# CHAINNEVERLIU/Pytorch-RL-EnhancedStableBaselines

Measured on AMD Instinct MI355X. Metric: env-steps/sec (SAC, two-series CSTR, 4096 vec-envs) at 1/2/4/8 GPUs, higher is better.
Workload: dtype f32; 1 GPU; SAC MlpPolicy class defaults on 4096 vectorised two-series CSTR envs per GPU (obs 4/act 2, euler, batch 256, ring 244x4096, 1 gradient step per vec-step; hipGraph replay, 8 iterations per graph); n_envs_per_gpu=4096, global_batch=256, parallelism=dp1, hip_graph=True, hip_graph_requested=True, graph_unroll=8, blas=rocblas, n_updates=2370

## Files before the change

### pytorch-rl-enhancedstablebaselines_amd/csrc/cstr_chain.hip

```cpp
#include <hip/hip_runtime.h>
#include <stdint.h>

#include "../../include/cstr_rl_hip.h"
#include "cstr_device.h"
#include "cstr_rng_device.h"

namespace {

using f32x4 = __attribute__((ext_vector_type(4))) float;
typedef unsigned int u32x4 __attribute__((ext_vector_type(4)));
constexpr int BUF_OOB = 0x40000000;
constexpr int CH_THREADS = 256, CH_WAVES = 4;
constexpr float LOG_STD_MIN = -20.0f, LOG_STD_MAX = 2.0f;
constexpr int MAX_A = CSTR_MAX_HEAD_ACT;

constexpr int SM_PART = 0;
constexpr int SM_RED = SM_PART + 3 * 64 * 4;
constexpr int SM_XS = SM_RED + 4 * 16 * 8;
constexpr int SM_GS = SM_XS + 16 * 16;
constexpr int SM_PANEL = SM_GS + 16 * 8;
static size_t chain_lds_bytes(int k, int w1_pad) { return (size_t)(SM_PANEL + 16 * (k + 4) + w1_pad * k) * sizeof(float); }

__device__ __forceinline__ __amdgpu_buffer_rsrc_t rsrc_of(const float *base, const int64_t floats)
{
// ... 60 lines not shown
    const bool col_ok = k0 + r < K;
#pragma unroll
    for (int u = 0; u < NQ; ++u) {
        const int n = 16 * (ks + S * u) + 4 * h;
        const int wo = 4 * (n * K + k0 + r);
        bq[u].x = ld32(rw, (col_ok && n < N) ? wo : BUF_OOB);
        bq[u].y = ld32(rw, (col_ok && n + 1 < N) ? wo + 4 * K : BUF_OOB);
        bq[u].z = ld32(rw, (col_ok && n + 2 < N) ? wo + 8 * K : BUF_OOB);
        bq[u].w = ld32(rw, (col_ok && n + 3 < N) ? wo + 12 * K : BUF_OOB);
    }
}

template <int NQ>
__device__ __forceinline__ f32x4 tile_mma(const float *panel, const int ld, const int kdim, const float4 (&bq)[NQ], const int ks, const int S)
{
    const int lane = threadIdx.x & 63, r = lane & 15, h = lane >> 4;
    f32x4 acc0 = {0.0f, 0.0f, 0.0f, 0.0f}, acc1 = acc0, acc2 = acc0, acc3 = acc0;
    float4 av[NQ];
#pragma unroll
    for (int u = 0; u < NQ; ++u) {
        const int k = 16 * (ks + S * u) + 4 * h;
        av[u] = make_float4(0.0f, 0.0f, 0.0f, 0.0f);
        if (k < kdim) av[u] = *reinterpret_cast<const float4 *>(panel + r * ld + k);
    }
#pragma unroll
    for (int u = 0; u < NQ; ++u) {
        if (16 * (ks + S * u) < kdim) {
            acc0 = __builtin_amdgcn_mfma_f32_16x16x4f32(av[u].x, bq[u].x, acc0, 0, 0, 0);
            acc1 = __builtin_amdgcn_mfma_f32_16x16x4f32(av[u].y, bq[u].y, acc1, 0, 0, 0);
            acc2 = __builtin_amdgcn_mfma_f32_16x16x4f32(av[u].z, bq[u].z, acc2, 0, 0, 0);
            acc3 = __builtin_amdgcn_mfma_f32_16x16x4f32(av[u].w, bq[u].w, acc3, 0, 0, 0);
        }
    }
    return (acc0 + acc1) + (acc2 + acc3);
}

__device__ __forceinline__ f32x4 combine_split_k(f32x4 acc, float *smem, const int T, const int S)
{
    const int lane = threadIdx.x & 63, wave = threadIdx.x >> 6;
    f32x4 *part = reinterpret_cast<f32x4 *>(smem + SM_PART);
    if (S > 1) {
        if (wave >= T) part[(wave - T) * 64 + lane] = acc;
        lds_barrier();
        if (wave < T) {
            for (int v = 1; v < S; ++v) acc += part[(wave + T * v - T) * 64 + lane];
        }
    }
    return acc;
}

constexpr int MAX_PARTS = 16;
template <int NP>
__device__ __forceinline__ float sum_parts_n(const __amdgpu_buffer_rsrc_t rs, const int n, const int64_t stride, const int64_t at)
{
    float v[NP];
#pragma unroll
    for (int p = 0; p < NP; ++p) v[p] = ld32(rs, p < n ? (int)(4 * (p * stride + at)) : BUF_OOB);
    float s = v[0];
#pragma unroll
    for (int p = 1; p < NP; ++p) s += v[p];
    return s;
}

struct PartBatch {
    float v[8];
    const float *part; int n; int64_t stride, at, total;
    __device__ __forceinline__ void request(const float *part_, const int n_, const int64_t stride_, const int64_t at_, const int64_t total_)
    {
        part = part_; n = n_; stride = stride_; at = at_; total = total_;
        const __amdgpu_buffer_rsrc_t rs = rsrc_of(part, total);
#pragma unroll
        for (int p = 0; p < 8; ++p) v[p] = ld32(rs, (p < n && n <= 8) ? (int)(4 * (p * stride + at)) : BUF_OOB);
    }
    __device__ __forceinline__ float sum() const;
};

__device__ __forceinline__ float sum_parts(const float *part, const int n, const int64_t stride, const int64_t at, const int64_t total_floats)
{
    const __amdgpu_buffer_rsrc_t rs = rsrc_of(part, total_floats);
    if (n <= 4) return sum_parts_n<4>(rs, n, stride, at);
    if (n <= 8) return sum_parts_n<8>(rs, n, stride, at);
    if (n <= MAX_PARTS) return sum_parts_n<MAX_PARTS>(rs, n, stride, at);
    float s = part[at];
    for (int p = 1; p < n; ++p) s += part[p * stride + at];
    return s;
}

__device__ __forceinline__ float PartBatch::sum() const
{
    if (n > 8) return sum_parts(part, n, stride, at, total);
    float s = v[0];
#pragma unroll
    for (int p = 1; p < 8; ++p) s += v[p];
    return s;
}

__device__ __forceinline__ void sample_action(const float mu, const float raw, const float e, float &a, float &lp_term)
{
    const float half_log_2pi = 0.91893853320467274178f;
    const float ls = fminf(fmaxf(raw, LOG_STD_MIN), LOG_STD_MAX);
    const float sd = expf(ls);
    const float u = mu + sd * e;
    a = tanhf(u);
    const float d = u - mu, var = sd * sd;
    lp_term = (-(d * d) / (2.0f * var) - logf(sd) - half_log_2pi) - logf(1.0f - a * a + 1e-6f);
}

template <int KIN>
constexpr int l1_pad() { return (KIN % 2 == 0 && KIN + 1 <= 16) ? 0 : (KIN + 1 <= 8 ? 8 : 16); }
template <int KIN>
constexpr bool l1_bias_in_k() { return KIN % 4 != 0; }

template <int KIN>
__device__ __forceinline__ float4 l1_direct_quad(const float *w1, const float *b1, const int n, const int h, float &bias)
{
    if (KIN % 4 == 0) {
        bias = b1[n];
        return 4 * h < KIN ? *reinterpret_cast<const float4 *>(w1 + (int64_t)n * KIN + 4 * h) : make_float4(0.0f, 0.0f, 0.0f, 0.0f);
    }
    bias = 0.0f;
    const int k0 = 4 * h;
    float2 lo = make_float2(0.0f, 0.0f), hi = lo;
    if (k0 + 1 < KIN) lo = *reinterpret_cast<const float2 *>(w1 + (int64_t)n * KIN + k0);
    else if (k0 == KIN) lo = make_float2(b1[n], 0.0f);
    if (k0 + 3 < KIN) hi = *reinterpret_cast<const float2 *>(w1 + (int64_t)n * KIN + k0 + 2);
    else if (k0 + 2 == KIN) hi = make_float2(b1[n], 0.0f);
    return make_float4(lo.x, lo.y, hi.x, hi.y);
}

template <int KIN>
__device__ __forceinline__ void stage_w1(float *w1s, const float *w1, const float *b1, const int h1)
{
    constexpr int KP = l1_pad<KIN>();
    if (KP == 0) return;
    for (int c = threadIdx.x; c < h1; c += CH_THREADS) {
        float w[KP > 0 ? KP : 4];
#pragma unroll
        for (int k = 0; k < KP; ++k) w[k] = k < KIN ? w1[(int64_t)c * KIN + k] : 0.0f;
        w[KP > 0 ? KIN : 0] = b1[c];
#pragma unroll
        for (int q = 0; q < KP / 4; ++q) *reinterpret_cast<float4 *>(w1s + c * KP + 4 * q) = make_float4(w[4 * q], w[4 * q + 1], w[4 * q + 2], w[4 * q + 3]);
    }
}

template <int KIN>
struct L1Direct {
    float4 wb[4];
    float bias[4];
    __device__ __forceinline__ void request(const float *w1, const float *b1, const int h1)
    {
        const int lane = threadIdx.x & 63, wave = threadIdx.x >> 6, r = lane & 15, h = lane >> 4;
#pragma unroll
        for (int i = 0; i < 4; ++i) wb[i] = l1_direct_quad<KIN>(w1, b1, min(16 * (wave + CH_WAVES * i) + r, h1 - 1), h, bias[i]);
    }
};

template <int KP, int KIN>
__device__ __forceinline__ void layer1_mfma(const float *xs, const float *w1s, float *panel, const int ld, const int h1,
                                            const L1Direct<KIN> *dir = nullptr, const float *w1 = nullptr, const float *b1 = nullptr)
{
    const int lane = threadIdx.x & 63, wave = threadIdx.x >> 6, r = lane & 15, h = lane >> 4;
    const bool hk = KP == 0 ? 4 * h < KIN + (l1_bias_in_k<KIN>() ? 1 : 0) : 4 * h < KP;
    const float4 zero4 = make_float4(0.0f, 0.0f, 0.0f, 0.0f);
    const float4 xa = hk ? *reinterpret_cast<const float4 *>(xs + r * 16 + 4 * h) : zero4;
    const int n_tiles = (h1 + 15) / 16;
    for (int t0 = wave; t0 < n_tiles; t0 += 4 * CH_WAVES) {
        float4 wb[4];
        float bb[4] = {0.0f, 0.0f, 0.0f, 0.0f};
#pragma unroll
        for (int i = 0; i < 4; ++i) {
            if (KP == 0) {
                if (t0 == wave) { wb[i] = dir->wb[i]; bb[i] = dir->bias[i]; }
                else wb[i] = l1_direct_quad<KIN>(w1, b1, min(16 * (t0 + CH_WAVES * i) + r, h1 - 1), h, bb[i]);
            } else {
                wb[i] = hk ? *reinterpret_cast<const float4 *>(w1s + min(16 * (t0 + CH_WAVES * i) + r, h1 - 1) * KP + 4 * h) : zero4;
            }
        }
        f32x4 acc0[4], acc1[4];
#pragma unroll
        for (int i = 0; i < 4; ++i) {
            acc0[i] = {0.0f, 0.0f, 0.0f, 0.0f};
            acc1[i] = acc0[i];
            acc0[i] = __builtin_amdgcn_mfma_f32_16x16x4f32(xa.x, wb[i].x, acc0[i], 0, 0, 0);
            acc1[i] = __builtin_amdgcn_mfma_f32_16x16x4f32(xa.y, wb[i].y, acc1[i], 0, 0, 0);
        }
#pragma unroll
        for (int i = 0; i < 4; ++i) {
            acc0[i] = __builtin_amdgcn_mfma_f32_16x16x4f32(xa.z, wb[i].z, acc0[i], 0, 0, 0);
            acc1[i] = __builtin_amdgcn_mfma_f32_16x16x4f32(xa.w, wb[i].w, acc1[i], 0, 0, 0);
        }
#pragma unroll
        for (int i = 0; i < 4; ++i) {
            const int tl = t0 + CH_WAVES * i;
            const f32x4 acc = acc0[i] + acc1[i];
            if (tl < n_tiles && 16 * tl + r < h1) {
#pragma unroll
                for (int e = 0; e < 4; ++e) panel[(4 * h + e) * ld + 16 * tl + r] = fmaxf(acc[e] + bb[i], 0.0f);
            }
        }
    }
}

__device__ __forceinline__ void store_panel(const float *panel, const int ld, float *out, const int width, const int m0)
{
    const int qpr = width / 4;
    for (int i = threadIdx.x; i < 16 * qpr; i += CH_THREADS) {
        const int row = i / qpr, q = i % qpr;
        *reinterpret_cast<float4 *>(out + (int64_t)(m0 + row) * width + 4 * q) = *reinterpret_cast<const float4 *>(panel + row * ld + 4 * q);
    }
}

struct ActorFwdArgs {
    cstr_sac_actor_t net;
    cstr_ring_t ring; int64_t *ring_ctl; int advance_ring;
    const int32_t *idx; int batch, tiles;
    float *x_data, *x_pi, *x_next, *out_done, *out_rew, *a_h1, *a_h2, *head_part;
    const uint64_t *head_rng_ctl; uint64_t head_rng_offset; float *eps_all;
    int rows_mode, head_n;
};

template <int D, int A, int NQ, int WX>
__global__ __launch_bounds__(CH_THREADS) void sac_actor_chain_fwd_kernel(const ActorFwdArgs a)
{
    extern __shared__ __align__(16) float smem[];
    constexpr int W = D + A, QPR = D / 4;
    const int t = threadIdx.x, lane = t & 63, wave = t >> 6, r = lane & 15, h = lane >> 4;
    const int T = WX ? exact_tiles<NQ, WX>() : a.tiles, S = CH_WAVES / T, tile = wave % T, ks = wave / T;
    const int H1 = WX ? exact_h1<WX>() : a.net.h1, H2 = WX ? exact_h2<WX>() : a.net.h2, B = a.batch, mode = a.rows_mode, HN = a.head_n;
    const int M = mode == CSTR_CHAIN_ROWS_PAIR ? 2 * B : B;
    const int n0 = (blockIdx.x * T + tile) * 16, m0 = blockIdx.y * 16;
    float *xs = smem + SM_XS, *red = smem + SM_RED, *panel = smem + SM_PANEL;
    const int ld = H1 + 4;
    float *w1s = panel + 16 * ld;
    const bool col_ok = n0 + r < H2;
    CH_STAMP(0, 0);
    float4 bq[NQ];
    load_b_fwd<NQ>(bq, a.net.w2, H2, H1, n0, ks, S);
    const int col = min(n0 + r, H2 - 1);
    const float bv = a.net.b2[col];
    float hwv[2 * A];
#pragma unroll
    for (int j = 0; j < 2 * A; ++j) hwv[j] = j < HN ? a.net.hw[(int64_t)j * H2 + col] : 0.0f;
    stage_w1<D>(w1s, a.net.w1, a.net.b1, H1);
    L1Direct<D> l1d;
    if (l1_pad<D>() == 0) l1d.request(a.net.w1, a.net.b1, H1);
    const bool mat = a.idx != nullptr && blockIdx.x == 0;
    float4 v = make_float4(0.0f, 0.0f, 0.0f, 0.0f), vo = v;
    float actv[A], dn = 0.0f, to = 0.0f, rw = 0.0f;
#pragma unroll
    for (int j = 0; j < A; ++j) actv[j] = 0.0f;
    int b = 0;
    bool next = false;
    const bool data_row = mode != CSTR_CHAIN_ROWS_PAIR;
    if (t < 16 * QPR) {
        const int row = t / QPR, qd = t % QPR, m = m0 + row;
        next = mode == CSTR_CHAIN_ROWS_PAIR ? m >= B : mode == CSTR_CHAIN_ROWS_NEXT;
        b = (mode == CSTR_CHAIN_ROWS_PAIR && next) ? m - B : m;
        if (a.idx) {
            const int64_t o = (int64_t)a.idx[b] * a.ring.n_envs + a.idx[B + b];
            v = *reinterpret_cast<const float4 *>((next ? a.ring.next_obs : a.ring.obs) + o * D + 4 * qd);
            if (mat && data_row && next) vo = *reinterpret_cast<const float4 *>(a.ring.obs + o * D + 4 * qd);
            if (mat && (!next || data_row) && qd == 0) {
#pragma unroll
                for (int j = 0; j < A; ++j) actv[j] = a.ring.act[o * A + j];
                dn = a.ring.done[o]; to = a.ring.timeout[o]; rw = a.ring.rew[o];
            }
        } else {
            const float2 *src = reinterpret_cast<const float2 *>((next ? a.x_next : a.x_pi) + (int64_t)b * W + 4 * qd);
            const float2 lo = src[0], hi = src[1];
            v = make_float4(lo.x, lo.y, hi.x, hi.y);
        }
        *reinterpret_cast<float4 *>(xs + row * 16 + 4 * qd) = v;
    } else if (t >= 64 && t < 64 + 16 * (4 - QPR)) {
        const int i = t - 64, row = i / (4 - QPR), qd = QPR + i % (4 - QPR);
        *reinterpret_cast<float4 *>(xs + row * 16 + 4 * qd) = make_float4(qd == QPR ? 1.0f : 0.0f, 0.0f, 0.0f, 0.0f);
    }
    constexpr int PAIRS = (A + 1) / 2;
    float e0 = 0.0f, e1 = 0.0f;
    const bool noise = a.eps_all != nullptr && blockIdx.x == 0 && wave == 3 && lane < 16 * PAIRS;
    if (noise) {
        const int row = lane / PAIRS, pr = lane % PAIRS;
        const uint64_t seed = a.head_rng_ctl[0], ctr = a.head_rng_ctl[1] + a.head_rng_offset + (uint64_t)(m0 + row);
        uint32_t rr[4];
        philox4x32_10((uint32_t)ctr, (uint32_t)(ctr >> 32), (uint32_t)pr, 0u, (uint32_t)seed, (uint32_t)(seed >> 32), rr);
        box_muller(rr[0], rr[1], e0, e1);
    }
    CH_STAMP(0, 1);
    lds_barrier();
    CH_STAMP(0, 2);
    layer1_mfma<l1_pad<D>(), D>(xs, w1s, panel, ld, H1, &l1d, a.net.w1, a.net.b1);
    lds_barrier();
    CH_STAMP(0, 3);
    f32x4 acc = tile_mma<NQ>(panel, ld, H1, bq, ks, S);
    CH_STAMP(0, 4);
    acc = combine_split_k(acc, smem, T, S);
    CH_STAMP(0, 5);
    float hv[4] = {0.0f, 0.0f, 0.0f, 0.0f};
    if (wave < T) {
#pragma unroll
        for (int e = 0; e < 4; ++e) hv[e] = col_ok ? fmaxf(acc[e] + bv, 0.0f) : 0.0f;
#pragma unroll
        for (int j = 0; j < 2 * A; ++j) {
            if (j < HN) {
#pragma unroll
                for (int e = 0; e < 4; ++e) {
                    const float s = rowsum16(hv[e] * hwv[j]);
// ... 786 lines not shown
#pragma unroll
        for (int e = 0; e < 4; ++e) d[e] = (col_ok && ty[e] > 0.0f) ? acc[e] : 0.0f;
        if (GACT) {
#pragma unroll
            for (int j = 0; j < A; ++j) {
#pragma unroll
                for (int e = 0; e < 4; ++e) {
                    const float s = rowsum16(d[e] * w1a[j]);
                    if (r == 0) red[(tile * 16 + 4 * h + e) * 8 + j] = s;
                }
            }
        }
    }
    if (GACT) {
        lds_barrier();
        if (t < 16 * A) {
            const int row = t / A, j = t % A;
            float s = red[row * 8 + j];
#pragma unroll
            for (int tl = 1; tl < T; ++tl) s += red[(tl * 16 + row) * 8 + j];
            o_gact[(((int64_t)g * gridDim.x + blockIdx.x) * B + m0 + row) * A + j] = s;
        }
    }
    CH_STAMP(2, 6);
    if (!GACT) {
        if (wave < T && col_ok) {
#pragma unroll
            for (int e = 0; e < 4; ++e) o_dz1[((int64_t)g * B + m0 + 4 * h + e) * H1 + k0 + r] = d[e];
        }
        const int cpg = (H2 + gridDim.x - 1) / gridDim.x;
        if (t / cpg == (int)blockIdx.x) {
#pragma unroll
            for (int row = 0; row < 16; ++row) o_dz2[((int64_t)g * B + m0 + row) * H2 + t] = y[row];
        }
    }
    if (t < 16 && blockIdx.x == 0) {
        const int row = m0 + t;
        if (o_q) o_q[(int64_t)g * B + row] = o_qv;
        if (o_gqp) o_gqp[(int64_t)g * B + row] = o_gq;
        if (MODE == 1 && g == 0 && o_tqp) o_tqp[row] = o_tq;
    }
    CH_STAMP(2, 7);
}

struct ActorBwdArgs {
    cstr_sac_actor_t net;
    const float *gact_part; int n_nets, n_parts; const float *ent_coef;
    const float *x_pi, *params, *eps, *a_h1, *a_h2;
    float *g_params, *dz2, *dz1;
    int batch, tiles, kind;
};

template <int D, int A, int NQ, int WX>
__global__ __launch_bounds__(CH_THREADS) void sac_actor_chain_bwd_kernel(const ActorBwdArgs a)
{
    extern __shared__ __align__(16) float smem[];
    constexpr int W = D + A;
    const int t = threadIdx.x, lane = t & 63, wave = t >> 6, r = lane & 15, h = lane >> 4;
    const int T = WX ? exact_tiles<NQ, WX>() : a.tiles, S = CH_WAVES / T, tile = wave % T, ks = wave / T;
    const int H1 = WX ? exact_h1<WX>() : a.net.h1, H2 = WX ? exact_h2<WX>() : a.net.h2, B = a.batch;
    const int k0 = (blockIdx.x * T + tile) * 16, m0 = blockIdx.y * 16;
    const bool col_ok = k0 + r < H1, det = a.kind == CSTR_CHAIN_HEAD_DETERMINISTIC;
    const int col = min(k0 + r, H1 - 1), HN = det ? A : 2 * A;
    float *gs = smem + SM_GS, *panel = smem + SM_PANEL;
    const int ld = H2 + 4;
    CH_STAMP(3, 0);
    float4 bq[NQ];
    load_b_bwd<NQ>(bq, a.net.w2, H2, H1, k0, ks, S);
    float ty[4];
#pragma unroll
    for (int e = 0; e < 4; ++e) ty[e] = a.a_h1[(int64_t)(m0 + 4 * h + e) * H1 + col];
    constexpr int ZT = 4;
    const int n_ztiles = (H2 + 15) / 16;
    float zb0[ZT], zb1[ZT], zm[ZT][4];
#pragma unroll
    for (int i = 0; i < ZT; ++i) {
        const int cc = min(16 * (wave + CH_WAVES * i) + r, H2 - 1);
        zb0[i] = h < HN ? a.net.hw[(int64_t)h * H2 + cc] : 0.0f;
        zb1[i] = HN > 4 ? a.net.hw[(int64_t)(4 + h) * H2 + cc] : 0.0f;
#pragma unroll
        for (int e = 0; e < 4; ++e) zm[i][e] = a.a_h2[(int64_t)(m0 + 4 * h + e) * H2 + cc];
    }
    float o_gu = 0.0f, o_gls = 0.0f;
    if (t < 16 * A) {
        const int row = t / A, j = t % A, b = m0 + row;
        const float av = a.x_pi[(int64_t)b * W + D + j];
        const float ecv = det ? 0.0f : a.ent_coef[0], raw = det ? 0.0f : a.params[(int64_t)b * 2 * A + A + j];
        const float epv = det ? 0.0f : a.eps[(int64_t)b * A + j];
        const int np = a.n_nets * a.n_parts;
        const float ga = sum_parts(a.gact_part, np, (int64_t)B * A, (int64_t)b * A + j, (int64_t)np * B * A);
        const float one_m = 1.0f - av * av;
        if (det) {
            o_gu = ga * one_m;
        } else {
            const float gl = ecv * (1.0f / (float)B);
            const float s = expf(fminf(fmaxf(raw, LOG_STD_MIN), LOG_STD_MAX));
            o_gu = ga * one_m + gl * (2.0f * av * one_m / (one_m + 1e-6f));
            o_gls = (raw >= LOG_STD_MIN && raw <= LOG_STD_MAX) ? o_gu * epv * s - gl : 0.0f;
        }
        gs[row * 8 + j] = o_gu;
        gs[row * 8 + A + j] = o_gls;
    }
    CH_STAMP(3, 1);
    lds_barrier();
    CH_STAMP(3, 2);
    {
        const bool two = HN > 4;
        const float ga0 = gs[r * 8 + h], ga1 = two ? gs[r * 8 + 4 + h] : 0.0f;
        const int cpg = (H2 + gridDim.x - 1) / gridDim.x;
        auto dz2_tile = [&](const int tl, const float hb0, const float hb1, const float (&m)[4]) {
            const int c = 16 * tl + r;
            f32x4 acc = {0.0f, 0.0f, 0.0f, 0.0f};
            acc = __builtin_amdgcn_mfma_f32_16x16x4f32(ga0, hb0, acc, 0, 0, 0);
            if (two) acc = __builtin_amdgcn_mfma_f32_16x16x4f32(ga1, hb1, acc, 0, 0, 0);
            const bool mine = c / cpg == (int)blockIdx.x;
            if (tl < n_ztiles && c < H2) {
#pragma unroll
                for (int e = 0; e < 4; ++e) {
                    const float dv = m[e] > 0.0f ? acc[e] : 0.0f;
                    panel[(4 * h + e) * ld + c] = dv;
                    if (mine) a.dz2[(int64_t)(m0 + 4 * h + e) * H2 + c] = dv;
                }
            }
        };
#pragma unroll
        for (int i = 0; i < ZT; ++i) dz2_tile(wave + CH_WAVES * i, zb0[i], zb1[i], zm[i]);
        for (int tl = wave + CH_WAVES * ZT; tl < n_ztiles; tl += CH_WAVES) {
            const int cc = min(16 * tl + r, H2 - 1);
            const float hb0 = h < HN ? a.net.hw[(int64_t)h * H2 + cc] : 0.0f, hb1 = two ? a.net.hw[(int64_t)(4 + h) * H2 + cc] : 0.0f;
            float m[4];
#pragma unroll
            for (int e = 0; e < 4; ++e) m[e] = a.a_h2[(int64_t)(m0 + 4 * h + e) * H2 + cc];
            dz2_tile(tl, hb0, hb1, m);
        }
    }
    lds_barrier();
    CH_STAMP(3, 3);
    f32x4 acc = tile_mma<NQ>(panel, ld, H2, bq, ks, S);
    CH_STAMP(3, 4);
    acc = combine_split_k(acc, smem, T, S);
    CH_STAMP(3, 5);
    if (wave < T && col_ok) {
#pragma unroll
        for (int e = 0; e < 4; ++e) a.dz1[(int64_t)(m0 + 4 * h + e) * H1 + k0 + r] = ty[e] > 0.0f ? acc[e] : 0.0f;
    }
    if (t < 16 * A && blockIdx.x == 0) {
        const int row = t / A, j = t % A, b = m0 + row;
        a.g_params[(int64_t)b * HN + j] = o_gu;
        if (!det) a.g_params[(int64_t)b * HN + A + j] = o_gls;
    }
    CH_STAMP(3, 7);
}

__global__ __launch_bounds__(256) void chain_sum_parts_kernel(const float *__restrict__ part, const int n_parts, const int64_t rows, const int cols,
                                                              float *__restrict__ out, const int64_t out_stride)
{
    const int64_t i = blockIdx.x * (int64_t)blockDim.x + threadIdx.x, n = rows * cols;
    if (i >= n) return;
    out[(i / cols) * out_stride + i % cols] = sum_parts(part, n_parts, n, i, (int64_t)n_parts * n);
}

static int nq_for(int kdim, int tiles, int nq_max = 16)
{
    const int s = CH_WAVES / tiles, nch = (kdim + 15) / 16, per = (nch + s - 1) / s;
    return per <= 4 ? 4 : per <= 8 ? 8 : per <= 16 ? 16 : (per <= 32 && nq_max >= 32) ? 32 : 0;
}

static bool chain_dims_ok(int h1, int h2, int64_t batch, int tiles)
{
    return h1 >= 16 && h2 >= 16 && h1 <= CSTR_CHAIN_MAX_WIDTH && h2 <= CSTR_CHAIN_MAX_WIDTH && h1 % 4 == 0 && h2 % 4 == 0 && batch >= 16 &&
           batch <= 1024 && batch % 16 == 0 && (tiles == 1 || tiles == 2 || tiles == 4);
}

static int chain_layout(int obs_dim, int act_dim)
{
    return (obs_dim == 4 && act_dim == 2) ? 0 : (obs_dim == 8 && act_dim == 2) ? 1 : (obs_dim == 8 && act_dim == 4) ? 2 : -1;
}

#define CHAIN_NQ(KERNEL, D_, A_, WX_, NQV, GRID, LDS, STREAM, ARGS)                                \
    do {                                                                                           \
        if ((NQV) == 4) KERNEL<D_, A_, 4, WX_><<<GRID, CH_THREADS, LDS, STREAM>>>(ARGS);           \
        else if ((NQV) == 8) KERNEL<D_, A_, 8, WX_><<<GRID, CH_THREADS, LDS, STREAM>>>(ARGS);      \
        else if ((NQV) == 16) KERNEL<D_, A_, 16, WX_><<<GRID, CH_THREADS, LDS, STREAM>>>(ARGS);    \
        else KERNEL<D_, A_, NQ_TOP_##KERNEL, 0><<<GRID, CH_THREADS, LDS, STREAM>>>(ARGS);          \
    } while (0)
#define NQ_TOP_sac_actor_chain_fwd_kernel 32
#define NQ_TOP_q_chain_fwd_kernel 32
#define NQ_TOP_q_chain_bwd_kernel 16
#define NQ_TOP_sac_actor_chain_bwd_kernel 16
#define CHAIN_DISPATCH(KERNEL, LAY, WXV, NQV, GRID, LDS, STREAM, ARGS)                             \
    do {                                                                                           \
        if ((LAY) == 0 && (WXV) == 1) CHAIN_NQ(KERNEL, 4, 2, 1, NQV, GRID, LDS, STREAM, ARGS);     \
        else if ((LAY) == 0 && (WXV) == 2) CHAIN_NQ(KERNEL, 4, 2, 2, NQV, GRID, LDS, STREAM, ARGS); \
        else if ((LAY) == 0) CHAIN_NQ(KERNEL, 4, 2, 0, NQV, GRID, LDS, STREAM, ARGS);              \
        else if ((LAY) == 1 && (WXV) == 1) CHAIN_NQ(KERNEL, 8, 2, 1, NQV, GRID, LDS, STREAM, ARGS); \
        else if ((LAY) == 1) CHAIN_NQ(KERNEL, 8, 2, 0, NQV, GRID, LDS, STREAM, ARGS);              \
        else if ((WXV) == 2) CHAIN_NQ(KERNEL, 8, 4, 2, NQV, GRID, LDS, STREAM, ARGS);              \
        else CHAIN_NQ(KERNEL, 8, 4, 0, NQV, GRID, LDS, STREAM, ARGS);                              \
    } while (0)

static int chain_wx(int h1, int h2, int tiles, int nq)
{
    static const bool off = getenv("CSTR_EXACT_SHAPES") && atoi(getenv("CSTR_EXACT_SHAPES")) == 0;
    if (off || (nq != 4 && nq != 8 && nq != 16)) return 0;
    if (h1 == 256 && h2 == 256 && nq == 4 * tiles) return 1;
    if (h1 == 400 && h2 == 300 && nq == 8 * tiles) return 2;
    return 0;
}

constexpr size_t CHAIN_LDS_LIMIT = 64 * 1024;

int chain_lean_enabled = 1;

struct QFwdLeanScalars { int batch, parts; const float *head_part, *hb, *eps; int part_rows, next_offset; float sigma, clip; unsigned long long roles; };

template <int D, int A, int NQ, int FIN, int PB>
void q_fwd_lean_go(const dim3 grid, const size_t lds, hipStream_t s, const QFwdLeanScalars &c, const QFwdLeanArgs &a)
{
    q_chain_fwd_lean_kernel<D, A, NQ, FIN, PB><<<grid, CH_THREADS, lds, s>>>(c.batch, c.parts, c.head_part, c.hb, c.eps, c.part_rows, c.next_offset, c.sigma,
                                                                             c.clip, c.roles, a);
}
template <int D, int A, int NQ>
void q_fwd_lean_variant(const int finv, const int pb, const dim3 grid, const size_t lds, hipStream_t s, const QFwdLeanScalars &c, const QFwdLeanArgs &a)
{
    if (finv == QF_PLAIN) q_fwd_lean_go<D, A, NQ, QF_PLAIN, 8>(grid, lds, s, c, a);
    else if (finv == QF_GAUSSIAN && pb == 8) q_fwd_lean_go<D, A, NQ, QF_GAUSSIAN, 8>(grid, lds, s, c, a);
    else if (finv == QF_GAUSSIAN) q_fwd_lean_go<D, A, NQ, QF_GAUSSIAN, 16>(grid, lds, s, c, a);
    else if (pb == 8) q_fwd_lean_go<D, A, NQ, QF_DETERMINISTIC, 8>(grid, lds, s, c, a);
    else q_fwd_lean_go<D, A, NQ, QF_DETERMINISTIC, 16>(grid, lds, s, c, a);
}
template <int D, int A, typename... Rest>
void q_fwd_lean_nq(const int nq, Rest &&...rest)
{
    if (nq == 4) q_fwd_lean_variant<D, A, 4>(rest...);
    else if (nq == 8) q_fwd_lean_variant<D, A, 8>(rest...);
    else q_fwd_lean_variant<D, A, 16>(rest...);
}

enum { QB_TD_ALPHA = 0, QB_TD_LOGP = 1, QB_TD_PLAIN = 2, QB_ACTOR_SAC = 3, QB_ACTOR_NEG_MEAN = 4 };
struct QBwdLeanScalars { int batch, parts; const float *qp[4]; };

template <int D, int A, int NQ, int MODE, bool ALPHA, bool NLOGP, int LB>
void q_bwd_lean_go(const dim3 grid, const size_t lds, hipStream_t s, const QBwdLeanScalars &c, const QBwdLeanArgs &a)
{
    q_chain_bwd_lean_kernel<D, A, NQ, MODE, ALPHA, NLOGP, LB><<<grid, CH_THREADS, lds, s>>>(c.batch, c.parts, c.qp[0], c.qp[1], c.qp[2], c.qp[3], a);
}
template <int D, int A, int NQ, int LB>
void q_bwd_lean_variant(const int variant, const dim3 grid, const size_t lds, hipStream_t s, const QBwdLeanScalars &c, const QBwdLeanArgs &a)
{
    if (variant == QB_TD_ALPHA) q_bwd_lean_go<D, A, NQ, 1, true, true, LB>(grid, lds, s, c, a);
    else if (variant == QB_TD_LOGP) q_bwd_lean_go<D, A, NQ, 1, false, true, LB>(grid, lds, s, c, a);
    else if (variant == QB_TD_PLAIN) q_bwd_lean_go<D, A, NQ, 1, false, false, LB>(grid, lds, s, c, a);
    else if (variant == QB_ACTOR_SAC) q_bwd_lean_go<D, A, NQ, 2, false, false, LB>(grid, lds, s, c, a);
    else q_bwd_lean_go<D, A, NQ, 3, false, false, LB>(grid, lds, s, c, a);
}
template <int D, int A, int NQ, typename... Rest>
void q_bwd_lean_lb(const int lb, Rest &&...rest)
{
    if (lb == 4) q_bwd_lean_variant<D, A, NQ, 4>(rest...);
    else if (lb == 8) q_bwd_lean_variant<D, A, NQ, 8>(rest...);
    else q_bwd_lean_variant<D, A, NQ, 16>(rest...);
}
template <int D, int A, typename... Rest>
void q_bwd_lean_nq(const int nq, Rest &&...rest)
{
    if (nq == 4) q_bwd_lean_lb<D, A, 4>(rest...);
    else if (nq == 8) q_bwd_lean_lb<D, A, 8>(rest...);
    else q_bwd_lean_lb<D, A, 16>(rest...);
}

bool q_fwd_lean_launch(const QFwdArgs &g, const int lay, const int wx, const int nq, const dim3 grid, const size_t lds, hipStream_t s)
{
    if (!chain_lean_enabled || wx != 1 || (lay != 0 && lay != 1)) return false;
    if (g.has_fin && g.fin.n_parts > MAX_PARTS) return false;
    QFwdLeanArgs a = {};
    QFwdLeanScalars c = {};
    c.batch = g.batch;
    for (int i = 0; i < g.n_nets; ++i) {
        a.nets[i] = g.nets[i];
        c.roles |= (unsigned long long)(g.nets[i].role & 15) << (4 * i);
    }
    int finv = QF_PLAIN, pb = 8;
    if (g.has_fin) {
        const cstr_sac_head_fin_t &f = g.fin;
        finv = f.kind == CSTR_CHAIN_HEAD_DETERMINISTIC ? QF_DETERMINISTIC : QF_GAUSSIAN;
        pb = part_bucket_row(f.n_parts);
        c.parts = f.n_parts; c.head_part = f.head_part; c.hb = f.hb; c.eps = f.eps; c.part_rows = f.part_rows; c.next_offset = f.next_offset;
        c.sigma = f.sigma; c.clip = f.clip;
        a.x_pi = f.x_pi; a.x_next = f.x_next; a.params = f.params; a.logp_pi = f.logp_pi; a.logp_next = f.logp_next;
    }
    if (lay == 0) q_fwd_lean_nq<4, 2>(nq, finv, pb, grid, lds, s, c, a);
    else q_fwd_lean_nq<8, 2>(nq, finv, pb, grid, lds, s, c, a);
    return true;
}

bool q_bwd_lean_launch(const QBwdArgs &g, const int lay, const int wx, const int nq, const dim3 grid, const size_t lds, hipStream_t s)
{
    const cstr_chain_root_t &rt = g.root;
    if (!chain_lean_enabled || wx != 1 || (lay != 0 && lay != 1) || rt.n_parts > MAX_PARTS) return false;
    const bool stores_dz = g.dz1 && g.dz2 && !g.gact_part, stores_gact = g.gact_part && !g.dz1 && !g.dz2;
    const bool alpha = rt.alpha.log_alpha != nullptr, nlogp = rt.next_logp != nullptr;
    int variant;
    if (rt.mode == 1) {
        if (!stores_dz || (alpha && !nlogp) || (!alpha && nlogp && !rt.ent_coef)) return false;
        variant = alpha ? QB_TD_ALPHA : nlogp ? QB_TD_LOGP : QB_TD_PLAIN;
    } else {
        if (!stores_gact) return false;
        variant = rt.mode == 2 ? QB_ACTOR_SAC : QB_ACTOR_NEG_MEAN;
    }
    QBwdLeanArgs a = {};
    QBwdLeanScalars c = {};
    for (int i = 0; i < g.n_nets; ++i) a.nets[i] = QBwdLeanNet{g.nets[i].w1, g.nets[i].w2, g.nets[i].w3, g.nets[i].h1, g.nets[i].h2};
    for (int q = 0; q < 4; ++q) { a.b3[q] = rt.b3[q]; c.qp[q] = rt.q_part[q]; }
    a.ec_src = alpha ? rt.alpha.log_alpha : rt.ent_coef;
    a.dz2 = g.dz2; a.dz1 = g.dz1; a.gact_part = g.gact_part; a.q_out = rt.q_out; a.gq_out = rt.gq_out; a.target_out = rt.target_out;
    a.gamma = rt.gamma; a.scale = rt.scale;
    a.root = rt;
    a.rew = rt.rew; a.done = rt.done; a.next_logp = rt.next_logp;
    c.batch = rt.batch; c.parts = rt.n_parts;
    const int lb = part_bucket_loss(rt.n_parts);
    if (lay == 0) q_bwd_lean_nq<4, 2>(nq, lb, variant, grid, lds, s, c, a);
    else q_bwd_lean_nq<8, 2>(nq, lb, variant, grid, lds, s, c, a);
    return true;
}

}

#ifdef CSTR_CHAIN_STAMPS
extern "C" int cstr_diag_chain_stamps(unsigned long long *host_out, int64_t words)
{
    return (int)hipMemcpyFromSymbol(host_out, HIP_SYMBOL(chain_stamps), (size_t)words * 8);
}
#endif

static int check_actor(const cstr_sac_actor_t *n)
{
    if (!n || !n->w1 || !n->b1 || !n->w2 || !n->b2 || !n->hw || !n->hb) return CSTR_E_BADARG;
    if (!((n->obs_dim == 4 && n->act_dim == 2) || (n->obs_dim == 8 && (n->act_dim == 2 || n->act_dim == 4)))) return CSTR_E_UNSUPPORTED;
    if (!aligned16(n->w1) || !aligned16(n->w2)) return CSTR_E_BADARG;
    return CSTR_OK;
}

extern "C" int cstr_sac_actor_chain_fwd_f32(const cstr_sac_actor_t *actor, const cstr_ring_t *ring, int64_t *ring_ctl, int advance_ring,
                                            const int32_t *sample_idx, int64_t batch, float *x_data, float *x_pi, float *x_next,
                                            float *out_done, float *out_rew, float *a_h1, float *a_h2, float *head_part,
                                            const uint64_t *head_rng_ctl, uint64_t head_rng_offset, float *eps_all, int rows_mode,
                                            int head_n, int tiles, cstr_stream_t stream)
{
    const int rc = check_actor(actor);
    if (rc) return rc;
    if (!head_part || (eps_all && !head_rng_ctl)) return CSTR_E_BADARG;
    if (rows_mode < CSTR_CHAIN_ROWS_PAIR || rows_mode > CSTR_CHAIN_ROWS_OBS || (head_n != actor->act_dim && head_n != 2 * actor->act_dim)) return CSTR_E_BADARG;
    if ((rows_mode != CSTR_CHAIN_ROWS_OBS && !x_next) || (rows_mode != CSTR_CHAIN_ROWS_NEXT && !x_pi)) return CSTR_E_BADARG;
    if (!chain_dims_ok(actor->h1, actor->h2, batch, tiles)) return CSTR_E_UNSUPPORTED;
    if ((x_pi && !aligned8(x_pi)) || (x_next && !aligned8(x_next))) return CSTR_E_BADARG;
    ActorFwdArgs a = {};
    a.net = *actor;
    if (sample_idx) {
        if (!ring || !ring->obs || !ring->next_obs || !ring->act || !ring->rew || !ring->done || !ring->timeout || !x_data || !out_done || !out_rew)
            return CSTR_E_BADARG;
        if (ring->obs_dim != actor->obs_dim || ring->act_dim != actor->act_dim) return CSTR_E_BADARG;
        if (advance_ring && !ring_ctl) return CSTR_E_BADARG;
        if (!aligned16(ring->obs) || !aligned16(ring->next_obs) || !aligned8(x_data)) return CSTR_E_BADARG;
        if (ring->rows >= 0xFFFFFFFFLL || ring->n_envs >= 0xFFFFFFFFLL) return CSTR_E_UNSUPPORTED;
        a.ring = *ring;
    }
    a.ring_ctl = ring_ctl; a.advance_ring = advance_ring;
    a.idx = sample_idx; a.batch = (int)batch; a.tiles = tiles;
    a.x_data = x_data; a.x_pi = x_pi; a.x_next = x_next; a.out_done = out_done; a.out_rew = out_rew;
    a.a_h1 = a_h1; a.a_h2 = a_h2; a.head_part = head_part; a.head_rng_ctl = head_rng_ctl; a.head_rng_offset = head_rng_offset; a.eps_all = eps_all;
    a.rows_mode = rows_mode; a.head_n = head_n;
    const dim3 grid((unsigned)((actor->h2 + 16 * tiles - 1) / (16 * tiles)), (unsigned)((rows_mode == CSTR_CHAIN_ROWS_PAIR ? 2 : 1) * batch / 16));
    const size_t lds = chain_lds_bytes(actor->h1, 0);
    const int nq = nq_for(actor->h1, tiles, 32), lay = chain_layout(actor->obs_dim, actor->act_dim);
    if (!nq || lds > CHAIN_LDS_LIMIT) return CSTR_E_UNSUPPORTED;
    hipStream_t s = (hipStream_t)stream;
    CHAIN_DISPATCH(sac_actor_chain_fwd_kernel, lay, chain_wx(actor->h1, actor->h2, tiles, nq), nq, grid, lds, s, a);
    return (int)hipGetLastError();
}

extern "C" int cstr_q_chain_fwd_f32(const cstr_chain_net_t *nets, int n_nets, int w_in, int obs_dim, int h1, int h2, int64_t batch,
                                    const cstr_sac_head_fin_t *fin, int tiles, cstr_stream_t stream)
{
    if (!nets || n_nets < 1 || n_nets > CSTR_CHAIN_MAX_NETS || w_in < 1 || w_in > 12 || obs_dim < 1 || obs_dim >= w_in) return CSTR_E_BADARG;
    if (!chain_dims_ok(h1, h2, batch, tiles)) return CSTR_E_UNSUPPORTED;
    QFwdArgs a = {};
    for (int g = 0; g < n_nets; ++g) {
        const cstr_chain_net_t &n = nets[g];
        if (!n.w1 || !n.b1 || !n.w2 || !n.b2 || !n.w3 || !n.b3 || !n.x || !n.q_part || !aligned16(n.w2)) return CSTR_E_BADARG;
        if (n.role < 0 || n.role > CSTR_CHAIN_ROLE_PI || (n.role != 0 && !fin)) return CSTR_E_BADARG;
        a.nets[g] = n;
    }
    if (fin) {
        if (!fin->head_part || !fin->hb || fin->n_parts < 1 || fin->act_dim < 1 || fin->act_dim > MAX_A || fin->obs_dim != obs_dim || fin->obs_dim + fin->act_dim != w_in)
            return CSTR_E_BADARG;
        const bool det = fin->kind == CSTR_CHAIN_HEAD_DETERMINISTIC;
        if (fin->kind != CSTR_CHAIN_HEAD_GAUSSIAN && !det) return CSTR_E_BADARG;
        if (fin->part_rows < batch || fin->next_offset < 0 || fin->next_offset + batch > fin->part_rows) return CSTR_E_BADARG;
        if (!det && (!fin->eps || !fin->x_pi || !fin->x_next || !fin->params || !fin->logp_pi || !fin->logp_next)) return CSTR_E_BADARG;
        for (int g = 0; g < n_nets; ++g) {
            const int role = nets[g].role;
            if ((role == CSTR_CHAIN_ROLE_NEXT_STORE && !fin->x_next) || ((role == CSTR_CHAIN_ROLE_STORE_PI || role == CSTR_CHAIN_ROLE_PI) && !fin->x_pi))
                return CSTR_E_BADARG;
        }
        a.fin = *fin;
        a.has_fin = 1;
    }
    a.n_nets = n_nets; a.h1 = h1; a.h2 = h2; a.batch = (int)batch; a.tiles = tiles;
    const dim3 grid((unsigned)((h2 + 16 * tiles - 1) / (16 * tiles)), (unsigned)(batch / 16), (unsigned)n_nets);
    const size_t lds = chain_lds_bytes(h1, (w_in % 2 == 0 && w_in + 1 <= 16) ? 0 : (w_in + 1 <= 8 ? 8 : 16));
    const int nq = nq_for(h1, tiles, 32), lay = chain_layout(obs_dim, w_in - obs_dim);
    if (!nq || lay < 0 || lds > CHAIN_LDS_LIMIT) return CSTR_E_UNSUPPORTED;
    hipStream_t s = (hipStream_t)stream;
    const int wx = chain_wx(h1, h2, tiles, nq);
    if (!q_fwd_lean_launch(a, lay, wx, nq, grid, lds, s)) CHAIN_DISPATCH(q_chain_fwd_kernel, lay, wx, nq, grid, lds, s, a);
    return (int)hipGetLastError();
}

extern "C" int cstr_q_chain_bwd_f32(const cstr_chain_net_t *nets, int n_nets, const cstr_chain_root_t *root, int w_in, int obs_dim, int h1,
                                    int h2, float *dz2, float *dz1, float *gact_part, int tiles, cstr_stream_t stream)
{
    if (!nets || !root || n_nets < 1 || n_nets > 2 || w_in < 1 || w_in > 12 || obs_dim < 0 || obs_dim > w_in) return CSTR_E_BADARG;
    if (root->mode < 1 || root->mode > 3 || root->n_parts < 1) return CSTR_E_BADARG;
    if ((root->mode == 3) != (n_nets == 1)) return CSTR_E_BADARG;
    if (!chain_dims_ok(h1, h2, root->batch, tiles)) return CSTR_E_UNSUPPORTED;
        QBwdArgs a = {};
    for (int g = 0; g < n_nets; ++g) {
        const cstr_chain_net_t &n = nets[g];
        if (!n.w1 || !n.w2 || !n.w3 || !n.h1 || !n.h2) return CSTR_E_BADARG;
        a.nets[g] = n;
    }
    const int need = root->mode == 1 ? 4 : n_nets;
    for (int g = 0; g < need; ++g)
        if (!root->q_part[g] || !root->b3[g]) return CSTR_E_BADARG;
    if (root->mode == 1 && (!root->rew || !root->done)) return CSTR_E_BADARG;
    if (root->mode == 2 && (!root->logp || !root->ent_coef)) return CSTR_E_BADARG;
    if (root->mode == 1 && root->alpha.log_alpha && (!root->alpha.logp_pi || !root->alpha.grad_out || !root->alpha.ent_coef_out)) return CSTR_E_BADARG;
    a.root = *root;
    a.n_nets = n_nets; a.h1 = h1; a.h2 = h2; a.tiles = tiles;
    a.dz2 = dz2; a.dz1 = dz1; a.gact_part = gact_part;
    const dim3 grid((unsigned)((h1 + 16 * tiles - 1) / (16 * tiles)), (unsigned)(root->batch / 16 + 1), (unsigned)n_nets);
    const size_t lds = chain_lds_bytes(h2, 0);
    const int nq = nq_for(h2, tiles), lay = chain_layout(obs_dim, w_in - obs_dim);
    if (!nq || lay < 0 || lds > CHAIN_LDS_LIMIT) return CSTR_E_UNSUPPORTED;
    hipStream_t s = (hipStream_t)stream;
    const int wx = chain_wx(h1, h2, tiles, nq);
    if (!q_bwd_lean_launch(a, lay, wx, nq, grid, lds, s)) CHAIN_DISPATCH(q_chain_bwd_kernel, lay, wx, nq, grid, lds, s, a);
    return (int)hipGetLastError();
}

extern "C" int cstr_chain_lean(int on)
{
    const int was = chain_lean_enabled;
    if (on >= 0) chain_lean_enabled = on != 0;
    return was;
}

extern "C" int cstr_chain_sum_parts_f32(const float *part, int n_parts, int64_t rows, int cols, float *out, int64_t out_stride, cstr_stream_t stream)
{
    if (!part || !out || n_parts < 1 || rows < 1 || cols < 1 || out_stride < cols) return CSTR_E_BADARG;
    if ((int64_t)n_parts * rows * cols >= (1 << 28)) return CSTR_E_UNSUPPORTED;
    const int64_t n = rows * cols;
    chain_sum_parts_kernel<<<(unsigned)((n + 255) / 256), 256, 0, (hipStream_t)stream>>>(part, n_parts, rows, cols, out, out_stride);
    return (int)hipGetLastError();
}

extern "C" int cstr_sac_actor_chain_bwd_f32(const cstr_sac_actor_t *actor, const float *gact_part, int n_nets, int n_parts,
                                            const float *ent_coef, const float *x_pi, const float *params, const float *eps, const float *a_h1,
                                            const float *a_h2, float *g_params, float *dz2, float *dz1, int64_t batch, int kind, int tiles,
                                            cstr_stream_t stream)
{
    const int rc = check_actor(actor);
    if (rc) return rc;
    if (kind != CSTR_CHAIN_HEAD_GAUSSIAN && kind != CSTR_CHAIN_HEAD_DETERMINISTIC) return CSTR_E_BADARG;
    if (!gact_part || n_nets < 1 || n_nets > 2 || n_parts < 1 || !x_pi || !a_h1 || !a_h2 || !g_params || !dz2 || !dz1) return CSTR_E_BADARG;
    if (kind == CSTR_CHAIN_HEAD_GAUSSIAN && (!ent_coef || !params || !eps)) return CSTR_E_BADARG;
    if (!chain_dims_ok(actor->h1, actor->h2, batch, tiles)) return CSTR_E_UNSUPPORTED;
    ActorBwdArgs a = {};
    a.net = *actor;
    a.gact_part = gact_part; a.n_nets = n_nets; a.n_parts = n_parts; a.ent_coef = ent_coef;
    a.x_pi = x_pi; a.params = params; a.eps = eps; a.a_h1 = a_h1; a.a_h2 = a_h2;
    a.g_params = g_params; a.dz2 = dz2; a.dz1 = dz1; a.batch = (int)batch; a.tiles = tiles; a.kind = kind;
    const dim3 grid((unsigned)((actor->h1 + 16 * tiles - 1) / (16 * tiles)), (unsigned)(batch / 16));
    const size_t lds = chain_lds_bytes(actor->h2, 0);
    const int nq = nq_for(actor->h2, tiles), lay = chain_layout(actor->obs_dim, actor->act_dim);
    if (!nq || lds > CHAIN_LDS_LIMIT) return CSTR_E_UNSUPPORTED;
    hipStream_t s = (hipStream_t)stream;
    CHAIN_DISPATCH(sac_actor_chain_bwd_kernel, lay, chain_wx(actor->h1, actor->h2, tiles, nq), nq, grid, lds, s, a);
    return (int)hipGetLastError();
}
```

Measured before the change: 72.80 million env-steps/s.

## Add lean specialised actor chain forward kernel with scalar args and templated variants

Adds a specialised actor forward chain kernel for the paired-rows, exact-width case. Gather and noise are compile-time template flags, and the rarely used pointers are packed into a separate args struct. Index, observation and RNG-control loads are issued early through buffer loads, and the layer-1 weight fetch is flattened for whole-quad rows. The aim is to cut register pressure, branching and load latency in a latency-bound small-batch kernel, at the cost of more template instantiations and code duplicated from the generic kernel.

```diff
diff --git a/pytorch-rl-enhancedstablebaselines_amd/csrc/cstr_chain.hip b/pytorch-rl-enhancedstablebaselines_amd/csrc/cstr_chain.hip
--- a/pytorch-rl-enhancedstablebaselines_amd/csrc/cstr_chain.hip
+++ b/pytorch-rl-enhancedstablebaselines_amd/csrc/cstr_chain.hip
@@ -236,6 +236,18 @@
         const int lane = threadIdx.x & 63, wave = threadIdx.x >> 6, r = lane & 15, h = lane >> 4;
 #pragma unroll
         for (int i = 0; i < 4; ++i) wb[i] = l1_direct_quad<KIN>(w1, b1, min(16 * (wave + CH_WAVES * i) + r, h1 - 1), h, bias[i]);
+    }
+    __device__ __forceinline__ void request_flat(const float *w1, const float *b1, const int h1)
+    {
+        static_assert(KIN % 4 == 0, "whole-quad rows only");
+        const int lane = threadIdx.x & 63, wave = threadIdx.x >> 6, r = lane & 15, h = lane >> 4;
+        const __amdgpu_buffer_rsrc_t rw = rsrc_of(w1, (int64_t)h1 * KIN);
+#pragma unroll
+        for (int i = 0; i < 4; ++i) {
+            const int n = min(16 * (wave + CH_WAVES * i) + r, h1 - 1);
+            bias[i] = b1[n];
+            wb[i] = ld128(rw, 4 * h < KIN ? 4 * (n * KIN + 4 * h) : BUF_OOB);
+        }
     }
 };
 
@@ -1328,6 +1340,171 @@
     CH_STAMP(3, 7);
 }
 
+typedef unsigned int u32x2 __attribute__((ext_vector_type(2)));
+
+struct ActorFwdLeanArgs {
+    const float *w1, *b1, *w2, *b2, *hw;
+    const float *ring_act, *ring_rew, *ring_done, *ring_timeout;
+    int64_t ring_rows; int64_t *ring_ctl; int advance_ring;
+    float *x_data, *out_done, *out_rew, *a_h1, *a_h2, *head_part, *eps_all;
+};
+
+template <int D, int A, int NQ, bool GATHER, bool NOISE>
+__global__ __launch_bounds__(CH_THREADS) void sac_actor_chain_fwd_lean_kernel(const int batch, const unsigned n_envs, const int32_t *idx, const float *ring_obs,
+                                                                              const float *ring_next, float *x_pi, float *x_next, const uint64_t *rng_ctl,
+                                                                              const uint64_t rng_offset, const ActorFwdLeanArgs a)
+{
+    extern __shared__ __align__(16) float smem[];
+    constexpr int W = D + A, QPR = D / 4, WX = 1, HN = 2 * A;
+    static_assert(l1_pad<D>() == 0 && D % 4 == 0, "whole-quad observation rows");
+    const int t = threadIdx.x, lane = t & 63, wave = t >> 6, r = lane & 15, h = lane >> 4;
+    constexpr int T = exact_tiles<NQ, WX>(), S = CH_WAVES / T;
+    const int tile = wave % T, ks = wave / T;
+    constexpr int H1 = exact_h1<WX>(), H2 = exact_h2<WX>();
+    const int B = batch, M = 2 * B;
+    const int n0 = (blockIdx.x * T + tile) * 16, m0 = blockIdx.y * 16;
+    float *xs = smem + SM_XS, *red = smem + SM_RED, *panel = smem + SM_PANEL;
+    constexpr int ld = H1 + 4;
+    float *w1s = panel + 16 * ld;
+    const bool col_ok = n0 + r < H2;
+    CH_STAMP(0, 0);
+    const bool gl = t < 16 * QPR, next = m0 >= B;
+    const int row = gl ? t / QPR : 0, qd = t % QPR;
+    const int b = (next ? m0 - B : m0) + row;
+    const bool mat = GATHER && blockIdx.x == 0;
+    unsigned ir = 0, ie = 0;
+    u32x2 plo = {0u, 0u}, phi = plo;
+    if (GATHER) {
+        const __amdgpu_buffer_rsrc_t ri = rsrc_of(reinterpret_cast<const float *>(idx), 2 * (int64_t)B);
+        ir = __builtin_amdgcn_raw_buffer_load_b32(ri, gl ? 4 * b : BUF_OOB, 0, 0);
+        ie = __builtin_amdgcn_raw_buffer_load_b32(ri, gl ? 4 * (B + b) : BUF_OOB, 0, 0);
+    } else {
+        const __amdgpu_buffer_rsrc_t rx = rsrc_of(next ? x_next : x_pi, (int64_t)B * W);
+        plo = __builtin_amdgcn_raw_buffer_load_b64(rx, gl ? 4 * (b * W + 4 * qd) : BUF_OOB, 0, 0);
+        phi = __builtin_amdgcn_raw_buffer_load_b64(rx, gl ? 4 * (b * W + 4 * qd) + 8 : BUF_OOB, 0, 0);
+    }
+    constexpr int PAIRS = (A + 1) / 2;
+    const bool noise = NOISE && blockIdx.x == 0 && wave == 3 && lane < 16 * PAIRS;
+    u32x2 c_seed = {0u, 0u}, c_ctr = c_seed;
+    if (NOISE) {
+        const __amdgpu_buffer_rsrc_t rc = rsrc_of(reinterpret_cast<const float *>(rng_ctl), 4);
+        c_seed = __builtin_amdgcn_raw_buffer_load_b64(rc, noise ? 0 : BUF_OOB, 0, 0);
+        c_ctr = __builtin_amdgcn_raw_buffer_load_b64(rc, noise ? 8 : BUF_OOB, 0, 0);
+    }
+    __builtin_amdgcn_sched_barrier(0);
+    const float *const w1 = a.w1, *const b1 = a.b1, *const w2 = a.w2, *const b2 = a.b2, *const hw = a.hw;
+    const float *const r_act = a.ring_act, *const r_rew = a.ring_rew, *const r_done = a.ring_done, *const r_timeout = a.ring_timeout;
+    const int64_t ring_rows = a.ring_rows;
+    int64_t *const ring_ctl = a.ring_ctl;
+    const int advance_ring = a.advance_ring;
+    float *const o_x_data = a.x_data, *const o_done = a.out_done, *const o_rew = a.out_rew, *const o_a_h1 = a.a_h1, *const o_a_h2 = a.a_h2;
+    float *const o_head_part = a.head_part, *const o_eps = a.eps_all;
+    asm volatile("" ::"s"(w1), "s"(b1), "s"(w2), "s"(b2), "s"(hw), "s"(o_a_h1), "s"(o_a_h2), "s"(o_head_part));
+    if (GATHER) asm volatile("" ::"s"(r_act), "s"(r_rew), "s"(r_done), "s"(r_timeout), "s"(ring_rows), "s"(ring_ctl), "s"(advance_ring), "s"(o_x_data), "s"(o_done), "s"(o_rew));
+    if (NOISE) asm volatile("" ::"s"(o_eps));
+    float4 bq[NQ];
+    load_b_fwd<NQ>(bq, w2, H2, H1, n0, ks, S);
+    const int col = min(n0 + r, H2 - 1);
+    const float bv = b2[col];
+    float hwv[HN];
+#pragma unroll
+    for (int j = 0; j < HN; ++j) hwv[j] = hw[(int64_t)j * H2 + col];
+    L1Direct<D> l1d;
+    l1d.request_flat(w1, b1, H1);
+    if (t >= 64 && t < 64 + 16 * (4 - QPR)) {
+        const int i = t - 64, prow = i / (4 - QPR), pq = QPR + i % (4 - QPR);
+        *reinterpret_cast<float4 *>(xs + prow * 16 + 4 * pq) = make_float4(pq == QPR ? 1.0f : 0.0f, 0.0f, 0.0f, 0.0f);
+    }
+    float4 v = make_float4(__uint_as_float(plo.x), __uint_as_float(plo.y), __uint_as_float(phi.x), __uint_as_float(phi.y));
+    float actv[A], dn = 0.0f, to = 0.0f, rw = 0.0f;
+#pragma unroll
+    for (int j = 0; j < A; ++j) actv[j] = 0.0f;
+    if (GATHER) {
+        const int64_t o = (int64_t)(int)ir * (int64_t)n_envs + (int)ie;
+        v = *reinterpret_cast<const float4 *>((next ? ring_next : ring_obs) + o * D + 4 * qd);
+        const int64_t od = (gl && mat && !next && qd == 0) ? o : 0;
+#pragma unroll
+        for (int j = 0; j < A; ++j) actv[j] = r_act[od * A + j];
+        dn = r_done[od]; to = r_timeout[od]; rw = r_rew[od];
+    }
+    if (gl) *reinterpret_cast<float4 *>(xs + row * 16 + 4 * qd) = v;
+    float e0 = 0.0f, e1 = 0.0f;
+    if (noise) {
+        const int nrow = lane / PAIRS, pr = lane % PAIRS;
+        const uint64_t seed = ((uint64_t)c_seed.y << 32) | c_seed.x, ctr = (((uint64_t)c_ctr.y << 32) | c_ctr.x) + rng_offset + (uint64_t)(m0 + nrow);
+        uint32_t rr[4];
+        philox4x32_10((uint32_t)ctr, (uint32_t)(ctr >> 32), (uint32_t)pr, 0u, (uint32_t)seed, (uint32_t)(seed >> 32), rr);
+        box_muller(rr[0], rr[1], e0, e1);
+    }
+    CH_STAMP(0, 1);
+    lds_barrier();
+    CH_STAMP(0, 2);
+    layer1_mfma<0, D>(xs, w1s, panel, ld, H1, &l1d, w1, b1);
+    lds_barrier();
+    CH_STAMP(0, 3);
+    f32x4 acc = tile_mma<NQ>(panel, ld, H1, bq, ks, S);
+    CH_STAMP(0, 4);
+    acc = combine_split_k(acc, smem, T, S);
+    CH_STAMP(0, 5);
+    float hv[4] = {0.0f, 0.0f, 0.0f, 0.0f};
+    if (wave < T) {
+#pragma unroll
+        for (int e = 0; e < 4; ++e) hv[e] = col_ok ? fmaxf(acc[e] + bv, 0.0f) : 0.0f;
+#pragma unroll
+        for (int j = 0; j < HN; ++j) {
+#pragma unroll
+            for (int e = 0; e < 4; ++e) {
+                const float s = rowsum16(hv[e] * hwv[j]);
+                if (r == 0) red[(tile * 16 + 4 * h + e) * 8 + j] = s;
+            }
+        }
+    }
+    lds_barrier();
+    CH_STAMP(0, 6);
+    if (t < 16 * HN) {
+        const int prow = t / HN, j = t % HN;
+        float s = red[prow * 8 + j];
+#pragma unroll
+        for (int tl = 1; tl < T; ++tl) s += red[(tl * 16 + prow) * 8 + j];
+        o_head_part[((int64_t)blockIdx.x * M + m0 + prow) * HN + j] = s;
+    }
+    const bool keep_rows = !next;
+    if (wave < T && col_ok && keep_rows) {
+#pragma unroll
+        for (int e = 0; e < 4; ++e) o_a_h2[(int64_t)(m0 + 4 * h + e) * H2 + n0 + r] = hv[e];
+    }
+    if (blockIdx.x == 0 && keep_rows) store_panel(panel, ld, o_a_h1, H1, m0);
+    if (noise) {
+        const int nrow = lane / PAIRS, pr = lane % PAIRS;
+        float *eo = o_eps + (int64_t)(m0 + nrow) * A + 2 * pr;
+        eo[0] = e0;
+        if (2 * pr + 1 < A) eo[1] = e1;
+    }
+    if (mat && gl) {
+        float *xo = (next ? x_next : x_pi) + (int64_t)b * W + 4 * qd;
+        reinterpret_cast<float2 *>(xo)[0] = make_float2(v.x, v.y); reinterpret_cast<float2 *>(xo)[1] = make_float2(v.z, v.w);
+        if (!next) {
+            float *xd = o_x_data + (int64_t)b * W;
+            reinterpret_cast<float2 *>(xd + 4 * qd)[0] = make_float2(v.x, v.y); reinterpret_cast<float2 *>(xd + 4 * qd)[1] = make_float2(v.z, v.w);
+            if (qd == 0) {
+#pragma unroll
+                for (int j = 0; j < A; ++j) xd[D + j] = actv[j];
+                o_done[b] = dn * (1.0f - to);
+                o_rew[b] = rw;
+            }
+        }
+    }
+    if (GATHER && blockIdx.x == 0 && blockIdx.y == 0 && t == 0) {
+        if (advance_ring) {
+            int64_t pos = ring_ctl[0] + 1;
+            if (pos == ring_rows) { ring_ctl[1] = 1; pos = 0; }
+            ring_ctl[0] = pos;
+            ring_ctl[3] += 1;
+        }
+    }
+    CH_STAMP(0, 7);
+}
+
 __global__ __launch_bounds__(256) void chain_sum_parts_kernel(const float *__restrict__ part, const int n_parts, const int64_t rows, const int cols,
                                                               float *__restrict__ out, const int64_t out_stride)
 {
@@ -1500,6 +1677,43 @@
     return true;
 }
 
+template <int D, int A, int NQ, bool GATHER, bool NOISE>
+void actor_fwd_lean_go(const dim3 grid, const size_t lds, hipStream_t s, const ActorFwdArgs &g, const ActorFwdLeanArgs &a)
+{
+    sac_actor_chain_fwd_lean_kernel<D, A, NQ, GATHER, NOISE><<<grid, CH_THREADS, lds, s>>>(g.batch, (unsigned)g.ring.n_envs, g.idx, g.ring.obs, g.ring.next_obs, g.x_pi,
+                                                                                          g.x_next, g.head_rng_ctl, g.head_rng_offset, a);
+}
+template <int D, int A, int NQ, typename... Rest>
+void actor_fwd_lean_variant(const bool gather, const bool noise, Rest &&...rest)
+{
+    if (gather && noise) actor_fwd_lean_go<D, A, NQ, true, true>(rest...);
+    else if (gather) actor_fwd_lean_go<D, A, NQ, true, false>(rest...);
+    else if (noise) actor_fwd_lean_go<D, A, NQ, false, true>(rest...);
+    else actor_fwd_lean_go<D, A, NQ, false, false>(rest...);
+}
+template <int D, int A, typename... Rest>
+void actor_fwd_lean_nq(const int nq, Rest &&...rest)
+{
+    if (nq == 4) actor_fwd_lean_variant<D, A, 4>(rest...);
+    else if (nq == 8) actor_fwd_lean_variant<D, A, 8>(rest...);
+    else actor_fwd_lean_variant<D, A, 16>(rest...);
+}
+
+bool actor_fwd_lean_launch(const ActorFwdArgs &g, const int lay, const int wx, const int nq, const dim3 grid, const size_t lds, hipStream_t s)
+{
+    if (!chain_lean_enabled || wx != 1 || (lay != 0 && lay != 1)) return false;
+    if (g.rows_mode != CSTR_CHAIN_ROWS_PAIR || g.head_n != 2 * g.net.act_dim || !g.a_h1 || !g.a_h2) return false;
+    ActorFwdLeanArgs a = {};
+    a.w1 = g.net.w1; a.b1 = g.net.b1; a.w2 = g.net.w2; a.b2 = g.net.b2; a.hw = g.net.hw;
+    a.ring_act = g.ring.act; a.ring_rew = g.ring.rew; a.ring_done = g.ring.done; a.ring_timeout = g.ring.timeout;
+    a.ring_rows = g.ring.rows; a.ring_ctl = g.ring_ctl; a.advance_ring = g.advance_ring;
+    a.x_data = g.x_data; a.out_done = g.out_done; a.out_rew = g.out_rew; a.a_h1 = g.a_h1; a.a_h2 = g.a_h2; a.head_part = g.head_part; a.eps_all = g.eps_all;
+    const bool gather = g.idx != nullptr, noise = g.eps_all != nullptr;
+    if (lay == 0) actor_fwd_lean_nq<4, 2>(nq, gather, noise, grid, lds, s, g, a);
+    else actor_fwd_lean_nq<8, 2>(nq, gather, noise, grid, lds, s, g, a);
+    return true;
+}
+
 }
 
 #ifdef CSTR_CHAIN_STAMPS
@@ -1551,7 +1765,8 @@
     const int nq = nq_for(actor->h1, tiles, 32), lay = chain_layout(actor->obs_dim, actor->act_dim);
     if (!nq || lds > CHAIN_LDS_LIMIT) return CSTR_E_UNSUPPORTED;
     hipStream_t s = (hipStream_t)stream;
-    CHAIN_DISPATCH(sac_actor_chain_fwd_kernel, lay, chain_wx(actor->h1, actor->h2, tiles, nq), nq, grid, lds, s, a);
+    const int wx = chain_wx(actor->h1, actor->h2, tiles, nq);
+    if (!actor_fwd_lean_launch(a, lay, wx, nq, grid, lds, s)) CHAIN_DISPATCH(sac_actor_chain_fwd_kernel, lay, wx, nq, grid, lds, s, a);
     return (int)hipGetLastError();
 }
 
```

After: 73.68 million env-steps/s, median of 6. 1.01x the previous value.
